# cc-ai/climategan

Hardware: AMD Instinct MI355X
Metric: 640x640 images/sec (G+D step): per-domain sample slots per second of the joint Masker+Painter training step (update_G + update_D), global batch 32 per domain (higher is better)
Workload: dtype bf16

## Files before the change

### climategan_amd/csrc/conv_wgrad.hip

```cpp
#include "cgan_common.h"
#include <type_traits>

namespace {


struct WgradArgs {
  const uint16_t* x;
  const uint16_t* dy;
  float* dw;
  unsigned x_bytes, dy_bytes;
  float* ws;
  float* bpart;
  int n, h_in, w_in, cin, cin_s;
  int cout, cout_s;
  int kh, kw, stride, pad, dil;
  int h_out, w_out, npix;
  int nchunks, ci_blocks, co_blocks, splits, per_xcd;
  int coop, co_pairs, n_pairs;
  int fold, cpt, tpt, tap_slots;
  CGAN_DEV_ONLY(int dbg;)
  int reflect;
  int x_ups;
  CGAN_DEV_ONLY(unsigned long long* ts;)
};
// ... 324 lines not shown
  const unsigned row_b = (unsigned)wx * cin_b;
  const wg_rsrc_t rs_x = wg_make_rsrc(p.x, p.x_bytes);
  const wg_rsrc_t rs_dy = wg_make_rsrc(p.dy, p.dy_bytes);
  unsigned dy_c = 0x80000000u;
  {
    const int co = (cop * G + mem) * 64 + q8;
    if ((cop * G + mem) < p.co_blocks && co < p.cout_s) dy_c = (unsigned)prow * cout_b + (unsigned)co * 2u;
  }
  int lx, ly;
  unsigned cch2, x_c;
  {
    int slot, cib, ky, kx, cch;
    bool ok = n_tile(mem, slot, cib);
    if (p.fold) {
      const int tl = qs / p.cpt, tap_l = slot * p.tpt + tl;
      ok = ok && tl < p.tpt && tap_l < taps_n;
      const int tcl = ok ? tap_l : 0;
      ky = tcl / p.kw;
      kx = tcl - ky * p.kw;
      cch = (qs - tl * p.cpt) * 8;
    } else {
      ky = slot / p.kw;
      kx = slot - ky * p.kw;
      cch = cib * 64 + q8;
      ok = ok && cch < p.cin_s;
    }
    const int tap_y = ky * p.dil - p.pad, tap_x = kx * p.dil - p.pad;
    const int lxr = prow * p.stride + tap_x;
    ly = tap_y;
    lx = ok ? lxr : -(1 << 20);
    cch2 = (unsigned)cch * 2u;
    x_c = (unsigned)((tap_y * wx + lxr) * (int)cin_b) + cch2;
  }

  int v_sx, v_sy, v_nh;
  {
    const int pix = split * CHUNK2 + (lane & (PPS - 1)) * 8;
    const int r = pix / p.w_out;
    v_sx = (pix - r * p.w_out) * p.stride;
    const int nn = r / p.h_out;
    v_sy = (r - nn * p.h_out) * p.stride;
    v_nh = nn * hx;
  }
  unsigned u_dy = (unsigned)(split * CHUNK2) * cout_b;
  const int step = p.splits * CHUNK2;
  const int step_r = step / p.w_out;
  const int step_sx = (step - step_r * p.w_out) * p.stride;
  const int step_n = step_r / p.h_out;
  const int step_sy = (step_r - step_n * p.h_out) * p.stride;
  const int step_nh = step_n * hx;
  const int wrap_x = p.w_out * p.stride, wrap_y = p.h_out * p.stride;
  const unsigned step_dy = (unsigned)step * cout_b;

  unsigned v_off = 0;
  auto issue_piece = [&](int b, int k) {
    unsigned char* dst = smem + b * STAGE2 + mem * SUB2 + half * (PW * PIECE);
    if (k < PW) {
      const unsigned off = u_dy + (unsigned)((half * PW + k) * 8) * cout_b + dy_c;
      wg_dma16(rs_dy, dst + k * PIECE, off);
      return;
    }
    const int j = k - PW, i = half * PW + j;
    if (j == 0) v_off = (unsigned)((v_nh + v_sy) * wx + v_sx) * cin_b;
    int iy = __builtin_amdgcn_readlane(v_sy, i) + ly, ix = __builtin_amdgcn_readlane(v_sx, i) + lx;
    if (MODE == 2) {
      iy = iy < 0 ? -iy : (iy >= p.h_in ? 2 * p.h_in - 2 - iy : iy);
      ix = ix < 0 ? -ix : (ix >= p.w_in ? 2 * p.w_in - 2 - ix : ix);
    }
    const bool xv = ((unsigned)iy < (unsigned)p.h_in) & ((unsigned)ix < (unsigned)p.w_in);
    unsigned off;
    if (MODE == 1) off = (unsigned)(__builtin_amdgcn_readlane(v_nh, i) + (iy >> 1)) * row_b + (unsigned)(ix >> 1) * cin_b + cch2;
    else if (MODE == 2) off = (unsigned)(__builtin_amdgcn_readlane(v_nh, i) + iy) * row_b + (unsigned)ix * cin_b + cch2;
    else off = (unsigned)__builtin_amdgcn_readlane((int)v_off, i) + x_c;
    wg_dma16(rs_x, dst + G * SUB2 + j * PIECE, xv ? off : 0xffffffffu);
  };
  auto advance = [&]() {
    u_dy += step_dy;
    int sx = v_sx + step_sx, sy = v_sy + step_sy, nh = v_nh + step_nh;
    const bool cx = sx >= wrap_x;
    sx = cx ? sx - wrap_x : sx;
    sy = cx ? sy + p.stride : sy;
    const bool cy = sy >= wrap_y;
    sy = cy ? sy - wrap_y : sy;
    nh = cy ? nh + hx : nh;
    v_sx = sx; v_sy = sy; v_nh = nh;
  };

  const int wc = wave % G, wn = wave / G;
  f32x4 acc[4][4];
#pragma unroll
  for (int a = 0; a < 4; ++a)
#pragma unroll
    for (int b = 0; b < 4; ++b) acc[a][b] = (f32x4){0.f, 0.f, 0.f, 0.f};

  const bool do_bias = BIAS && p.bpart != nullptr && np == 0 && wn == 0;
  f32x4 accb[4];
#pragma unroll
  for (int a = 0; a < 4; ++a) accb[a] = (f32x4){0.f, 0.f, 0.f, 0.f};
  const int nchunks = (p.npix + CHUNK2 - 1) / CHUNK2;
  int c = split, buf = 0;
  unsigned long long t_a = 0, t_b = 0, ts_sum[4] = {0, 0, 0, 0}, t_start = 0;
  if (TS) t_start = __builtin_readcyclecounter();
  if (c < nchunks) {
#pragma unroll
    for (int k = 0; k < 2 * PW; ++k) issue_piece(0, k);
    advance();
  }
  for (; c < nchunks; c += p.splits) {
    if (TS) t_a = __builtin_readcyclecounter();
    asm volatile("s_waitcnt vmcnt(0) lgkmcnt(0)" ::: "memory");
    if (TS) { t_b = __builtin_readcyclecounter(); ts_sum[0] += t_b - t_a; }
    __syncthreads();
    if (TS) { t_a = __builtin_readcyclecounter(); ts_sum[1] += t_a - t_b; }
    if (c + p.splits < nchunks) {
#pragma unroll
      for (int k = 0; k < 2 * PW; ++k) issue_piece(buf ^ 1, k);
      advance();
    }
    if (TS) { t_b = __builtin_readcyclecounter(); ts_sum[2] += t_b - t_a; }
    const unsigned char* sdy = smem + buf * STAGE2 + wc * SUB2;
    const unsigned char* sx = smem + buf * STAGE2 + (G + wn) * SUB2;
#pragma unroll
    for (int ks = 0; ks < CH / 32; ++ks) {
      u32x4 fa[4], fb[4];
#pragma unroll
      for (int a = 0; a < 4; ++a) fa[a] = tr_frag(sdy + ks * 4 * PIECE, a, lane);
#pragma unroll
      for (int b = 0; b < 4; ++b) fb[b] = tr_frag(sx + ks * 4 * PIECE, b, lane);
#pragma unroll
      for (int a = 0; a < 4; ++a)
#pragma unroll
        for (int b = 0; b < 4; ++b) acc[a][b] = mfma16(as_vec8<T>(fa[a]), as_vec8<T>(fb[b]), acc[a][b]);
      if (BIAS && do_bias) {
#pragma unroll
        for (int a = 0; a < 4; ++a) accb[a] = mfma16(as_vec8<T>(fa[a]), as_vec8<T>(ones_frag<T>()), accb[a]);
      }
    }
    buf ^= 1;
    if (TS) { t_a = __builtin_readcyclecounter(); ts_sum[3] += t_a - t_b; }
  }
  if (BIAS && do_bias && cop * G + wc < p.co_blocks)
    store_bias_row(p.bpart + (size_t)split * p.cout_s, accb, 4, (cop * G + wc) * 64, p.cout_s, lane);
  if (TS && CGAN_WTS(p) && lane == 0) {
    unsigned long long* o = CGAN_WTS(p) + ((size_t)blockIdx.x * (G * G) + wave) * 8;
    o[0] = t_start;
    o[1] = __builtin_readcyclecounter();
    for (int i = 0; i < 4; ++i) o[2 + i] = ts_sum[i];
    o[6] = (unsigned long long)((nchunks - split + p.splits - 1) / p.splits);
  }

  const int cob = cop * G + wc;
  int slot_c, cib_c;
  const bool nt_ok = n_tile(wn, slot_c, cib_c);
  if (cob >= p.co_blocks || !nt_ok) return;
  if (p.ws) {
    const int tiles_n = p.tap_slots * p.ci_blocks * p.co_blocks;
    const int tile = (slot_c * p.ci_blocks + cib_c) * p.co_blocks + cob;
    f32x4* wst = reinterpret_cast<f32x4*>(p.ws) + ((size_t)split * tiles_n + tile) * 1024;
#pragma unroll
    for (int a = 0; a < 4; ++a)
#pragma unroll
      for (int b = 0; b < 4; ++b) wst[(a * 4 + b) * 64 + lane] = acc[a][b];
    return;
  }
  const int j = lane & 15, g = lane >> 4;
#pragma unroll
  for (int b = 0; b < 4; ++b) {
    int tap, ci;
    const bool col_ok = wgrad_column(p.fold, p.cpt, p.tpt, taps_n, p.cin, slot_c, cib_c, b * 16 + j, tap, ci);
#pragma unroll
    for (int a = 0; a < 4; ++a)
#pragma unroll
      for (int r = 0; r < 4; ++r) {
        const int co = cob * 64 + a * 16 + 4 * g + r;
        if (co < p.cout && col_ok && !(CGAN_DBG(p) & 1)) atomicAdd(p.dw + ((size_t)co * p.cin + ci) * taps_n + tap, acc[a][b][r]);
      }
  }
}

constexpr int TL_W = 32, TL_H = 4, TL_XP = 40;
constexpr int TL_XH_BYTES = (TL_H + 2) * TL_XP * 128;
constexpr int TL_DY_BYTES = TL_H * TL_W * 128;

__device__ __forceinline__ u32x4 tr_frag_at(const unsigned char* slab, int q0, int tile, int lane) {
  const int i = lane & 15, g = lane >> 4;
  const int k = i >> 2;
  const int chunk = tile * 2 + ((i & 3) >> 1);
  const int qa = q0 + 8 * g + k, qb = qa + 4;
  const unsigned char* a0 = slab + qa * 128 + ((chunk ^ swz(qa & 7)) << 4) + (i & 1) * 8;
  const unsigned char* a1 = slab + qb * 128 + ((chunk ^ swz(qb & 7)) << 4) + (i & 1) * 8;
  s16x4 lo = __builtin_amdgcn_ds_read_tr16_b64_v4i16((__attribute__((address_space(3))) s16x4*)a0);
  s16x4 hi = __builtin_amdgcn_ds_read_tr16_b64_v4i16((__attribute__((address_space(3))) s16x4*)a1);
  u32x4 r;
  r[0] = (uint16_t)lo[0] | ((uint32_t)(uint16_t)lo[1] << 16);
  r[1] = (uint16_t)lo[2] | ((uint32_t)(uint16_t)lo[3] << 16);
  r[2] = (uint16_t)hi[0] | ((uint32_t)(uint16_t)hi[1] << 16);
  r[3] = (uint16_t)hi[2] | ((uint32_t)(uint16_t)hi[3] << 16);
  return r;
}

template <typename T, int NA = 4, bool BIAS = false>
__global__ __launch_bounds__(256, 2) void conv_wgrad_tile3x3_kernel(WgradArgs p) {
  extern __shared__ __attribute__((aligned(1024))) unsigned char smem[];
  unsigned char* xh = smem;
  unsigned char* dyt = smem + TL_XH_BYTES;
  const int lane = threadIdx.x & 63;
  const int wave = __builtin_amdgcn_readfirstlane(threadIdx.x >> 6);
  int item = (blockIdx.x & 7) * p.per_xcd + (blockIdx.x >> 3);
  if ((int)(blockIdx.x >> 3) >= p.per_xcd || item >= p.co_blocks * p.ci_blocks * p.splits) return;
  const int cob = item % p.co_blocks;
  item /= p.co_blocks;
  const int cib = item % p.ci_blocks;
  const int split = item / p.ci_blocks;

  const int prow = lane >> 3, qs = (lane & 7) ^ swz(prow);
  const unsigned cin_b = (unsigned)p.cin_s * 2u, cout_b = (unsigned)p.cout_s * 2u;
  const __amdgpu_buffer_rsrc_t rs_x = __builtin_amdgcn_make_buffer_rsrc(const_cast<uint16_t*>(p.x), 0, p.x_bytes, 0x00020000);
  const __amdgpu_buffer_rsrc_t rs_dy = __builtin_amdgcn_make_buffer_rsrc(const_cast<uint16_t*>(p.dy), 0, p.dy_bytes, 0x00020000);
  const bool ci_ok = cib * 64 + qs * 8 < p.cin_s, co_ok = cob * 64 + qs * 8 < p.cout_s;
  const unsigned x_c = (unsigned)(cib * 64 + qs * 8) * 2u, dy_c = (unsigned)(cob * 64 + qs * 8) * 2u;

  const int tw = p.w_out / TL_W, th = p.h_out / TL_H;
  const int ntiles = p.n * th * tw;

  auto stage = [&](int t) {
    const int tc = t % tw;
    const int r0 = t / tw;
    const int tr = r0 % th, img = r0 / th;
    const int ty0 = tr * TL_H, tx0 = tc * TL_W;
#pragma unroll
    for (int rr = 0; rr < 2; ++rr) {
      const int r = wave + 4 * rr;
      if (r < TL_H + 2) {
        const int iy = ty0 - 1 + r;
        const unsigned row_off = (unsigned)((img * p.h_in + iy) * p.w_in) * cin_b + x_c;
#pragma unroll
        for (int i5 = 0; i5 < 5; ++i5) {
          const int ix = tx0 - 4 + 8 * i5 + prow;
          const bool ok = ci_ok & ((unsigned)iy < (unsigned)p.h_in) & ((unsigned)ix < (unsigned)p.w_in);
          __builtin_amdgcn_raw_ptr_buffer_load_lds(rs_x, (__attribute__((address_space(3))) void*)(xh + (r * TL_XP + 8 * i5) * 128), 16,
                                                   ok ? row_off + (unsigned)ix * cin_b : 0xffffffffu, 0, 0, 0);
        }
      }
    }
    const int j0 = wave < 2 ? wave * 2 : 4 + (wave - 2) * 6, nj = wave < 2 ? 2 : 6;
#pragma unroll
    for (int jj = 0; jj < 6; ++jj) {
      if (jj < nj) {
        const int j = j0 + jj, r = j >> 2, c8 = (j & 3) * 8;
        const unsigned off = (unsigned)((img * p.h_out + ty0 + r) * p.w_out + tx0 + c8 + prow) * cout_b + dy_c;
        __builtin_amdgcn_raw_ptr_buffer_load_lds(rs_dy, (__attribute__((address_space(3))) void*)(dyt + (r * TL_W + c8) * 128), 16,
                                                 co_ok ? off : 0xffffffffu, 0, 0, 0);
      }
    }
  };

  f32x4 acc[NA][9];
#pragma unroll
  for (int a = 0; a < NA; ++a)
#pragma unroll
    for (int i = 0; i < 9; ++i) acc[a][i] = (f32x4){0.f, 0.f, 0.f, 0.f};

  const bool do_bias = BIAS && p.bpart != nullptr && cib == 0 && wave == 0;
  f32x4 accb[4];
#pragma unroll
  for (int a = 0; a < 4; ++a) accb[a] = (f32x4){0.f, 0.f, 0.f, 0.f};
  for (int t = split; t < ntiles; t += p.splits) {
    __syncthreads();
    stage(t);
    asm volatile("s_waitcnt vmcnt(0)" ::: "memory");
    __syncthreads();
#pragma unroll 1
    for (int ty = 0; ty < TL_H; ++ty) {
      u32x4 fa[NA];
#pragma unroll
      for (int a = 0; a < NA; ++a) fa[a] = tr_frag_at(dyt, ty * TL_W, a, lane);
      if (BIAS && do_bias) {
#pragma unroll
        for (int a = 0; a < NA; ++a) accb[a] = mfma16(as_vec8<T>(fa[a]), as_vec8<T>(ones_frag<T>()), accb[a]);
      }
#pragma unroll
      for (int i = 0; i < 9; ++i) {
        const int jn = wave * 9 + i, tap = jn >> 2, grp = jn & 3;
        const int ky = tap / 3, kx = tap - ky * 3;
        const u32x4 fb = tr_frag_at(xh, (ty + ky) * TL_XP + 3 + kx, grp, lane);
#pragma unroll
        for (int a = 0; a < NA; ++a) acc[a][i] = mfma16(as_vec8<T>(fa[a]), as_vec8<T>(fb), acc[a][i]);
      }
    }
  }

  if (BIAS && do_bias) store_bias_row(p.bpart + (size_t)split * p.cout_s, accb, NA, cob * 64, p.cout_s, lane);
  const int tiles_n = 9 * p.ci_blocks * p.co_blocks;
#pragma unroll
  for (int i = 0; i < 9; ++i) {
    const int jn = wave * 9 + i, tap = jn >> 2, grp = jn & 3;
    const int tile = (tap * p.ci_blocks + cib) * p.co_blocks + cob;
    f32x4* wst = reinterpret_cast<f32x4*>(p.ws) + ((size_t)split * tiles_n + tile) * 1024;
#pragma unroll
    for (int a = 0; a < 4; ++a) wst[(a * 4 + grp) * 64 + lane] = a < NA ? acc[a < NA ? a : 0][i] : (f32x4){0.f, 0.f, 0.f, 0.f};
  }
}

template <int KL>
__global__ __launch_bounds__(256) void wgrad_reduce_kernel(const f32x4* __restrict__ ws, float* __restrict__ dw,
                                                           int splits, int taps, int tap_slots, int ci_blocks,
                                                           int co_blocks, int cout, int cin, int fold, int cpt,
                                                           int tpt, int main_blocks, const float* __restrict__ bpart,
                                                           int bias_rows, int cout_s, float* __restrict__ dbias) {
  if ((int)blockIdx.x >= main_blocks) {
    __shared__ float bsum[16][17];
    const int c16 = (int)threadIdx.x & 15, rl = (int)threadIdx.x >> 4;
    const int ch = ((int)blockIdx.x - main_blocks) * 16 + c16;
    float a0 = 0.f, a1 = 0.f, a2 = 0.f, a3 = 0.f;
    if (ch < cout) {
      int r = rl;
      for (; r + 48 < bias_rows; r += 64) {
        a0 += bpart[(size_t)r * cout_s + ch];
        a1 += bpart[(size_t)(r + 16) * cout_s + ch];
        a2 += bpart[(size_t)(r + 32) * cout_s + ch];
        a3 += bpart[(size_t)(r + 48) * cout_s + ch];
      }
      for (; r < bias_rows; r += 16) a0 += bpart[(size_t)r * cout_s + ch];
    }
    bsum[rl][c16] = (a0 + a1) + (a2 + a3);
    __syncthreads();
    if (rl == 0 && ch < cout) {
      float acc = 0.f;
#pragma unroll
      for (int l = 0; l < 16; ++l) acc += bsum[l][c16];
      dbias[ch] += acc;
    }
    return;
  }
  constexpr int EL = 256 / KL;
  __shared__ f32x4 red[KL][EL];
  const int tiles_n = tap_slots * ci_blocks * co_blocks;
  const int el = threadIdx.x % EL, kl = threadIdx.x / EL;
  const int e = blockIdx.x * EL + el;
  f32x4 s = (f32x4){0.f, 0.f, 0.f, 0.f};
  if (e < tiles_n * 1024) {
    const size_t stride = (size_t)tiles_n * 1024;
#pragma unroll 4
    for (int sp = kl; sp < splits; sp += KL) {
      const f32x4 v = ws[(size_t)sp * stride + e];
      s[0] += v[0]; s[1] += v[1]; s[2] += v[2]; s[3] += v[3];
    }
  }
  if (KL > 1) {
    red[kl][el] = s;
    __syncthreads();
    if (kl != 0) return;
#pragma unroll
    for (int l = 1; l < KL; ++l) {
      const f32x4 v = red[l][el];
      s[0] += v[0]; s[1] += v[1]; s[2] += v[2]; s[3] += v[3];
    }
  }
  if (e >= tiles_n * 1024) return;
  int tile = e >> 10;
  const int frag = (e >> 6) & 15, lane = e & 63;
  const int cob = tile % co_blocks;
  tile /= co_blocks;
  const int cib = tile % ci_blocks, slot = tile / ci_blocks;
  int tap, ci;
  if (!wgrad_column(fold, cpt, tpt, taps, cin, slot, cib, (frag & 3) * 16 + (lane & 15), tap, ci)) return;
#pragma unroll
  for (int r = 0; r < 4; ++r) {
    const int co = cob * 64 + (frag >> 2) * 16 + 4 * (lane >> 4) + r;
    if (co >= cout) continue;
    dw[((size_t)co * cin + ci) * taps + tap] += s[r];
  }
}

template <typename T>
__global__ __launch_bounds__(256) void channel_sum_kernel(const uint16_t* __restrict__ x, float* __restrict__ out,
                                                          long npix, int cs, int c, float* __restrict__ part) {
  extern __shared__ __attribute__((aligned(16))) float sm_cs[];
  const int groups = cs / 8;
  const int ppb = blockDim.x / groups;
  const int gi = threadIdx.x % groups, pl = threadIdx.x / groups;
  float s[8] = {0.f, 0.f, 0.f, 0.f, 0.f, 0.f, 0.f, 0.f};
  if (pl < ppb) {
#pragma unroll 4
    for (long pix = (long)blockIdx.x * ppb + pl; pix < npix; pix += (long)gridDim.x * ppb) {
      const u32x4 v = *reinterpret_cast<const u32x4*>(x + pix * cs + gi * 8);
#pragma unroll
      for (int e = 0; e < 4; ++e) {
        float a, b;
        unpack2<T>(v[e], a, b);
        s[2 * e] += a;
        s[2 * e + 1] += b;
      }
    }
#pragma unroll
    for (int e = 0; e < 8; ++e) sm_cs[(pl * groups + gi) * 8 + e] = s[e];
  }
  __syncthreads();
  for (int ch = threadIdx.x; ch < groups * 8; ch += blockDim.x) {
    if (ch >= c) continue;
    float acc = 0.f;
    for (int l = 0; l < ppb; ++l) acc += sm_cs[l * groups * 8 + ch];
    if (part) part[(size_t)blockIdx.x * cs + ch] = acc;
    else atomicAdd(out + ch, acc);
  }
}

CGAN_KNOB(int, g_wgrad_target, 0);
CGAN_KNOB(int, g_wgrad_dbg, 0);
CGAN_KNOB(int, g_wgrad_coop_min_pix, 32768);
CGAN_KNOB(int, g_wgrad_coop_chunk, 0);
CGAN_KNOB(int, g_wgrad_slots, 512);
CGAN_KNOB(int, g_wgrad_tile, 1);
CGAN_KNOB(int, g_wgrad_coop_g, 0);
CGAN_KNOB(int, g_wgrad_bias_fused, 1);
CGAN_KNOB(int, g_wgrad_ws_cost_pct, 100);
CGAN_KNOB(unsigned long long*, g_wgrad_ts, nullptr);
}

#ifdef CGAN_DEV
extern "C" void cgan_debug_set_wgrad_tsbuf(void* p) { g_wgrad_ts = (unsigned long long*)p; }
extern "C" void cgan_debug_set_wgrad_bias_fused(int v) { g_wgrad_bias_fused = v; }
extern "C" void cgan_debug_set_wgrad_ws_cost(int pct) { g_wgrad_ws_cost_pct = pct > 0 ? pct : 100; }
extern "C" void cgan_debug_set_wgrad_tile3x3(int v) { g_wgrad_tile = v; }
extern "C" void cgan_debug_set_wgrad_slots(int v) { g_wgrad_slots = v > 0 ? v : 512; }
extern "C" void cgan_debug_set_wgrad_coop_chunk(int v) { g_wgrad_coop_chunk = (v == 32 || v == 64) ? v : 0; }

extern "C" void cgan_debug_set_wgrad_coop_min_pixels(int v) { g_wgrad_coop_min_pix = v; }
extern "C" void cgan_debug_set_wgrad_coop_g(int v) { g_wgrad_coop_g = (v == 2 || v == 4) ? v : 0; }

extern "C" void cgan_debug_set_wgrad(int target_workgroups, int dbg) {
  g_wgrad_target = target_workgroups;
  g_wgrad_dbg = dbg;
}
#endif

constexpr int BIAS_MAX_BLOCKS = 512;
constexpr int BIAS_MAX_ROWS = 1024;

struct WgradPlan {
  int fold, cpt, tpt, tap_slots, ci_blocks, co_blocks, splits;
  int coop, co_pairs, n_pairs, chunk;
  int g;
  int tile;
  long tiles() const { return (long)tap_slots * ci_blocks * co_blocks; }
};

static WgradPlan wgrad_plan(const CganConvDesc* d, bool have_ws = true) {
  WgradPlan pl;
  const int taps = d->kh * d->kw, cin_s = cgan_cs(d->c_in);
  pl.co_blocks = ceil_div(cgan_cs(d->c_out), 64);
  pl.fold = (cin_s <= 32 && taps > 1 && g_wgrad_dbg != 4) ? 1 : 0;
  pl.cpt = pl.fold ? cin_s / 8 : 8;
  pl.tpt = pl.fold ? 8 / pl.cpt : 1;
  pl.tap_slots = pl.fold ? ceil_div(taps, pl.tpt) : taps;
  pl.ci_blocks = pl.fold ? 1 : ceil_div(cin_s, 64);
  const long npix = (long)d->n * d->h_out * d->w_out;
  pl.g = 2;
  pl.co_pairs = (pl.co_blocks + 1) / 2;
  pl.n_pairs = pl.fold ? (pl.tap_slots + 1) / 2 : pl.tap_slots * ((pl.ci_blocks + 1) / 2);
  pl.coop = ((pl.co_blocks % 2) == 0 && ((pl.fold ? pl.tap_slots : pl.ci_blocks) % 2) == 0 && (d->w_out % 8) == 0 &&
             (g_wgrad_dbg & 8) == 0 && (double)npix * cgan_cs(d->c_out) * 2.0 < 1.9e9 &&
             (npix >= (long)g_wgrad_coop_min_pix || pl.tiles() >= 256))
                ? 1 : 0;
  pl.tile = ((g_wgrad_tile == 2 || (g_wgrad_tile == 1 && !pl.coop)) && have_ws && !pl.fold && d->kh == 3 && d->kw == 3 && d->stride == 1 && d->pad == 1 &&
             d->dilation == 1 && d->pad_mode == CGAN_PAD_ZERO && !d->in_upsample && (d->w_out % TL_W) == 0 &&
             (d->h_out % TL_H) == 0 && (cin_s % 64) == 0 && npix >= 65536 && (g_wgrad_dbg & (8 | 16)) == 0) ? 1 : 0;
  if (pl.tile) {
    pl.coop = 0;
    pl.chunk = TL_W * TL_H;
    const long pairs = (long)pl.co_blocks * pl.ci_blocks, ntiles = npix / (TL_W * TL_H);
    long sp = g_wgrad_target < 0 ? -g_wgrad_target : (long)g_wgrad_slots / pairs;
    if (sp > ntiles) sp = ntiles;
    pl.splits = sp < 1 ? 1 : (int)sp;
    return pl;
  }
  const long tiles = pl.coop ? (long)pl.co_pairs * pl.n_pairs : pl.tiles();
  auto plan_splits = [&](int chunk, long slots, int& nchunks_out) {
    const int nchunks = (int)((npix + chunk - 1) / chunk);
    nchunks_out = nchunks;
    long sp_best = 1;
    if (g_wgrad_target > 0) {
      sp_best = (g_wgrad_target + tiles - 1) / tiles;
    } else if (g_wgrad_target < 0) {
      sp_best = -g_wgrad_target;
    } else {
      const double t_ws = (pl.coop ? 0.024 : 0.008) * (g_wgrad_ws_cost_pct / 100.0);
      double best = 1e30;
      for (int m = 0; m <= 8; ++m) {
        long sp = m == 0 ? 1 : (slots * m) / tiles;
        if (sp < 1) continue;
        if (sp > nchunks) sp = nchunks;
        const long wgs = sp * tiles;
        const double cost = (double)((wgs + slots - 1) / slots) * ((double)((nchunks + sp - 1) / sp) + 2.0) + (double)wgs * t_ws;
        if (cost < best) { best = cost; sp_best = sp; }
      }
    }
    if (sp_best > nchunks) sp_best = nchunks;
    return sp_best < 1 ? 1L : sp_best;
  };
  int nchunks = 0;
  pl.chunk = pl.coop ? 64 : 128;
  if (pl.coop && g_wgrad_coop_g != 2 && (pl.co_blocks % 4) == 0 && ((pl.fold ? pl.tap_slots : pl.ci_blocks) % 4) == 0 &&
      g_wgrad_coop_chunk == 0) {
    const long tiles4 = (long)(pl.co_blocks / 4) * (pl.fold ? pl.tap_slots / 4 : (long)pl.tap_slots * (pl.ci_blocks / 4));
    const int nch = (int)((npix + 63) / 64);
    long sp = g_wgrad_target < 0 ? -g_wgrad_target : (g_wgrad_slots / 2) / tiles4;
    if (sp < 1) sp = 1;
    if (sp > nch) sp = nch;
    if (g_wgrad_coop_g == 4 || (tiles4 <= g_wgrad_slots / 2 && nch / sp >= 8)) {
      pl.g = 4;
      pl.co_pairs = pl.co_blocks / 4;
      pl.n_pairs = pl.fold ? pl.tap_slots / 4 : pl.tap_slots * (pl.ci_blocks / 4);
      pl.chunk = 64;
      pl.splits = (int)sp;
      return pl;
    }
  }
  long splits = plan_splits(pl.chunk, g_wgrad_slots, nchunks);
  if (pl.coop && (g_wgrad_coop_chunk == 32 || (g_wgrad_coop_chunk == 0 && nchunks / splits >= 96))) {
    pl.chunk = 32;
    splits = plan_splits(32, 2 * g_wgrad_slots, nchunks);
  }
  if (splits > nchunks) splits = nchunks;
  pl.splits = splits < 1 ? 1 : (int)splits;
  return pl;
}

extern "C" size_t cgan_conv2d_bwd_weight_workspace_bytes(const CganConvDesc* d) {
  if (!d || d->n <= 0 || d->h_out <= 0 || d->w_out <= 0 || d->c_in <= 0 || d->c_out <= 0 || d->kh <= 0 || d->kw <= 0)
    return 0;
  const WgradPlan pl = wgrad_plan(d);
  return (size_t)pl.tiles() * (size_t)pl.splits * 64 * 64 * sizeof(float) + (size_t)BIAS_MAX_ROWS * cgan_cs(d->c_out) * sizeof(float);
}

extern "C" int cgan_conv2d_nhwc_bwd_weight(const void* x, const void* dy, float* dw_oihw, float* dbias,
                                           const CganConvDesc* d, void* workspace, size_t workspace_bytes,
                                           void* stream) {
  CGAN_REQUIRE(d != nullptr && x && dy && dw_oihw, "conv2d_nhwc_bwd_weight: null pointer");
  CGAN_REQUIRE(d->dtype == CGAN_F16 || d->dtype == CGAN_BF16, "conv2d_nhwc_bwd_weight: bad dtype %d", d->dtype);
  CGAN_REQUIRE(d->pad_mode == CGAN_PAD_ZERO || d->pad_mode == CGAN_PAD_REFLECT, "conv2d_nhwc_bwd_weight: bad pad mode");
  if (d->pad_mode == CGAN_PAD_REFLECT)
    CGAN_REQUIRE(d->pad < d->h_in && d->pad < d->w_in && !d->in_upsample,
                 "conv2d_nhwc_bwd_weight: reflect padding must be < input size (and is not combined with in_upsample)");
  if (d->in_upsample) CGAN_REQUIRE((d->h_in % 2) == 0 && (d->w_in % 2) == 0, "conv2d_nhwc_bwd_weight: in_upsample needs even h_in/w_in");
  CGAN_REQUIRE(d->n > 0 && d->h_in > 0 && d->w_in > 0 && d->c_in > 0 && d->c_out > 0 && d->kh > 0 && d->kw > 0 &&
                   d->stride > 0 && d->dilation > 0 && d->pad >= 0,
               "conv2d_nhwc_bwd_weight: bad shape");
  const int eh = (d->h_in + 2 * d->pad - d->dilation * (d->kh - 1) - 1) / d->stride + 1;
  const int ew = (d->w_in + 2 * d->pad - d->dilation * (d->kw - 1) - 1) / d->stride + 1;
  CGAN_REQUIRE(eh == d->h_out && ew == d->w_out, "conv2d_nhwc_bwd_weight: h_out/w_out inconsistent");
  WgradArgs a;
  a.x = (const uint16_t*)x; a.dy = (const uint16_t*)dy; a.dw = dw_oihw;
  a.n = d->n; a.h_in = d->h_in; a.w_in = d->w_in; a.cin = d->c_in; a.cin_s = cgan_cs(d->c_in);
  a.cout = d->c_out; a.cout_s = cgan_cs(d->c_out);
  a.kh = d->kh; a.kw = d->kw; a.stride = d->stride; a.pad = d->pad; a.dil = d->dilation;
  a.h_out = d->h_out; a.w_out = d->w_out;
  const long npix = (long)d->n * d->h_out * d->w_out;
  CGAN_REQUIRE(npix < (1L << 31) - 256, "conv2d_nhwc_bwd_weight: too many pixels");
  a.npix = (int)npix;
  a.x_ups = d->in_upsample;
  a.reflect = d->pad_mode == CGAN_PAD_REFLECT;
  a.nchunks = ceil_div(a.npix, 128);
  const WgradPlan pl = wgrad_plan(d, workspace != nullptr);
  a.ci_blocks = pl.ci_blocks; a.co_blocks = pl.co_blocks; a.splits = pl.splits;
  a.fold = pl.fold; a.cpt = pl.cpt; a.tpt = pl.tpt; a.tap_slots = pl.tap_slots;
  a.coop = pl.coop; a.co_pairs = pl.co_pairs; a.n_pairs = pl.n_pairs;
  const int taps = d->kh * d->kw;
  CGAN_DEV_ONLY(a.dbg = g_wgrad_dbg; a.ts = g_wgrad_ts;)
  const long items = (long)a.splits * (pl.tile ? (long)pl.co_blocks * pl.ci_blocks
                                              : (pl.coop ? (long)pl.co_pairs * pl.n_pairs : pl.tiles()));
  a.per_xcd = (int)((items + 7) / 8);
  CGAN_REQUIRE(items < (1L << 30), "conv2d_nhwc_bwd_weight: grid too large");
  const unsigned gx = (unsigned)a.per_xcd * 8;
  a.ws = nullptr;
  a.bpart = nullptr;
  int bias_rows = 0;
  if (workspace) {
    CGAN_REQUIRE(workspace_bytes >= cgan_conv2d_bwd_weight_workspace_bytes(d),
                 "conv2d_nhwc_bwd_weight: workspace too small (%zu bytes)", workspace_bytes);
    a.ws = (float*)workspace;
    const int rows = a.splits * ((pl.tile || pl.coop) ? 1 : 4);
    const bool variant_ok = pl.tile ? (pl.co_blocks == 1 && ceil_div(cgan_cs(d->c_out), 16) < 4)
                                    : (!pl.coop || (pl.chunk == 64 && pl.g == 2));
    if (dbias && rows <= BIAS_MAX_ROWS && variant_ok && g_wgrad_bias_fused && CGAN_WTS(a) == nullptr) {
      a.bpart = a.ws + (size_t)pl.tiles() * (size_t)pl.splits * 64 * 64;
      bias_rows = rows;
    }
  }
  hipStream_t s = (hipStream_t)stream;
  const size_t smem = 4 * WAVE_LDS;
  CGAN_REQUIRE((double)d->n * (a.x_ups ? d->h_in / 2 : d->h_in) * (a.x_ups ? d->w_in / 2 : d->w_in) * a.cin_s * 2.0 < 4294967295.0 &&
                   (double)a.npix * a.cout_s * 2.0 < 4294967295.0,
               "conv2d_nhwc_bwd_weight: activation tensors of 4 GiB or more are not supported");
  a.x_bytes = (unsigned)((size_t)d->n * (a.x_ups ? d->h_in / 2 : d->h_in) * (a.x_ups ? d->w_in / 2 : d->w_in) * a.cin_s * 2);
  a.dy_bytes = (unsigned)((size_t)a.npix * a.cout_s * 2);
  const int mode = a.x_ups ? 1 : (a.reflect ? 2 : 0);
  const bool uni = (d->w_out % 8) == 0 && g_wgrad_dbg != 16 &&
                   ((double)a.npix + (double)a.splits * 128.0 + 128.0) * a.cout_s * 2.0 < 2147483648.0;
#define CGAN_BIG_LDS(KERNEL)                                                                                           \
  do {                                                                                                                 \
    static unsigned long long done_mask = 0;                                                                           \
    int dev_ = 0;                                                                                                      \
    (void)hipGetDevice(&dev_);                                                                                         \
    if (!((done_mask >> (dev_ & 63)) & 1ull)) {                                                                        \
      hipError_t e_ = hipFuncSetAttribute(reinterpret_cast<const void*>(&KERNEL),                                      \
                                          hipFuncAttributeMaxDynamicSharedMemorySize, 160 * 1024);                     \
      if (e_ != hipSuccess) {                                                                                          \
        cgan_set_error("conv2d_nhwc_bwd_weight: hipFuncSetAttribute failed: %s", hipGetErrorString(e_));               \
        return CGAN_ERR_HIP;                                                                                           \
      }                                                                                                                \
      done_mask |= 1ull << (dev_ & 63);                                                                                \
    }                                                                                                                  \
  } while (0)
#define WGRAD_LAUNCH(TT, MM, UU) do { CGAN_BIG_LDS((conv_wgrad_kernel<TT, MM, UU>)); hipLaunchKernelGGL((conv_wgrad_kernel<TT, MM, UU>), dim3(gx), dim3(256), smem, s, a); } while (0)
#define WGRAD_MODE(TT)                                                          \
  do {                                                                          \
    if (mode == 2) { if (uni) WGRAD_LAUNCH(TT, 2, true); else WGRAD_LAUNCH(TT, 2, false); }     \
    else if (mode == 1) { if (uni) WGRAD_LAUNCH(TT, 1, true); else WGRAD_LAUNCH(TT, 1, false); } \
    else { if (uni) WGRAD_LAUNCH(TT, 0, true); else WGRAD_LAUNCH(TT, 0, false); }                \
  } while (0)
  if (pl.tile) {
    const size_t smem3 = TL_XH_BYTES + TL_DY_BYTES;
    const int na = pl.co_blocks == 1 ? ceil_div(a.cout_s, 16) : 4;
#define TILE_LAUNCH(TT, NN, BB) hipLaunchKernelGGL((conv_wgrad_tile3x3_kernel<TT, NN, BB>), dim3(gx), dim3(256), smem3, s, a)
#define TILE_NB(TT, NN) do { if (a.bpart) TILE_LAUNCH(TT, NN, true); else TILE_LAUNCH(TT, NN, false); } while (0)
#define TILE_NA(TT) do { if (na == 1) TILE_NB(TT, 1); else if (na == 2) TILE_NB(TT, 2); else if (na == 3) TILE_NB(TT, 3); else TILE_LAUNCH(TT, 4, false); } while (0)
    if (d->dtype == CGAN_F16) TILE_NA(F16); else TILE_NA(BF16);
#undef TILE_NA
#undef TILE_NB
#undef TILE_LAUNCH
  } else if (pl.coop && pl.g == 4) {
    const size_t smem4 = (size_t)2 * 8 * 8 * PIECE;
#define COOP4_LAUNCH(TT, MM)                                                                                           \
  do {                                                                                                                 \
    CGAN_BIG_LDS((conv_wgrad_coop_kernel<TT, MM, 64, false, false, 4>));                                               \
    hipLaunchKernelGGL((conv_wgrad_coop_kernel<TT, MM, 64, false, false, 4>), dim3(gx), dim3(1024), smem4, s, a);      \
  } while (0)
#define COOP4_MODE(TT) do { if (mode == 1) COOP4_LAUNCH(TT, 1); else if (mode == 2) COOP4_LAUNCH(TT, 2); else COOP4_LAUNCH(TT, 0); } while (0)
#ifdef CGAN_DEV
    if (CGAN_WTS(a) && d->dtype == CGAN_BF16 && mode == 0) {
      CGAN_BIG_LDS((conv_wgrad_coop_kernel<BF16, 0, 64, true, false, 4>));
      hipLaunchKernelGGL((conv_wgrad_coop_kernel<BF16, 0, 64, true, false, 4>), dim3(gx), dim3(1024), smem4, s, a);
    } else
#endif
    if (d->dtype == CGAN_F16) COOP4_MODE(F16);
    else COOP4_MODE(BF16);
#undef COOP4_MODE
#undef COOP4_LAUNCH
  } else if (pl.coop) {
    const size_t smem2 = (size_t)2 * 4 * (pl.chunk / 8) * PIECE;
#define COOP_LAUNCH(TT, MM, CC, BB) do { CGAN_BIG_LDS((conv_wgrad_coop_kernel<TT, MM, CC, false, BB>)); hipLaunchKernelGGL((conv_wgrad_coop_kernel<TT, MM, CC, false, BB>), dim3(gx), dim3(256), smem2, s, a); } while (0)
#define COOP_MODE(TT)                                                                       \
  do {                                                                                      \
    if (pl.chunk == 32) { if (mode == 1) COOP_LAUNCH(TT, 1, 32, false); else if (mode == 2) COOP_LAUNCH(TT, 2, 32, false); else COOP_LAUNCH(TT, 0, 32, false); } \
    else if (a.bpart) { if (mode == 1) COOP_LAUNCH(TT, 1, 64, true); else if (mode == 2) COOP_LAUNCH(TT, 2, 64, true); else COOP_LAUNCH(TT, 0, 64, true); }            \
    else { if (mode == 1) COOP_LAUNCH(TT, 1, 64, false); else if (mode == 2) COOP_LAUNCH(TT, 2, 64, false); else COOP_LAUNCH(TT, 0, 64, false); }            \
  } while (0)
#ifdef CGAN_DEV
    if (CGAN_WTS(a) && d->dtype == CGAN_BF16 && mode == 0) {
      if (pl.chunk == 32) hipLaunchKernelGGL((conv_wgrad_coop_kernel<BF16, 0, 32, true>), dim3(gx), dim3(256), smem2, s, a);
      else { CGAN_BIG_LDS((conv_wgrad_coop_kernel<BF16, 0, 64, true>)); hipLaunchKernelGGL((conv_wgrad_coop_kernel<BF16, 0, 64, true>), dim3(gx), dim3(256), smem2, s, a); }
    } else
#endif
    if (d->dtype == CGAN_F16) COOP_MODE(F16);
    else COOP_MODE(BF16);
#undef COOP_MODE
#undef COOP_LAUNCH
  } else if (d->dtype == CGAN_F16) WGRAD_MODE(F16); else WGRAD_MODE(BF16);
#undef WGRAD_MODE
#undef WGRAD_LAUNCH
  CGAN_CHECK_LAUNCH("conv2d_nhwc_bwd_weight");
  float* bpart = a.bpart;
  if (dbias && !a.bpart) {
    const int cs = a.cout_s;
    const int threads = 256;
    const int ppb = threads / (cs / 8) > 0 ? threads / (cs / 8) : 1;
    CGAN_REQUIRE(cs / 8 <= threads, "conv2d_nhwc_bwd_weight: too many channels for the bias reduction");
    long want = (npix + (long)ppb * 16 - 1) / ((long)ppb * 16);
    const int grid = (int)(want < 1 ? 1 : (want > BIAS_MAX_BLOCKS ? BIAS_MAX_BLOCKS : want));
    const size_t smem_b = (size_t)ppb * (cs / 8) * 8 * sizeof(float);
    if (a.ws) {
      bpart = a.ws + (size_t)pl.tiles() * (size_t)pl.splits * 64 * 64;
      bias_rows = grid;
    }
    if (d->dtype == CGAN_F16)
      hipLaunchKernelGGL(channel_sum_kernel<F16>, dim3(grid), dim3(threads), smem_b, s, (const uint16_t*)dy, dbias, npix,
                         cs, d->c_out, bpart);
    else
      hipLaunchKernelGGL(channel_sum_kernel<BF16>, dim3(grid), dim3(threads), smem_b, s, (const uint16_t*)dy, dbias, npix,
                         cs, d->c_out, bpart);
    CGAN_CHECK_LAUNCH("conv2d_nhwc_bwd_weight(bias)");
  }
  if (a.ws) {
    const int elems = (int)pl.tiles() * 1024;
    const int bias_blocks = bpart ? ceil_div(d->c_out, 16) : 0;
    if (a.splits <= 4) {
      const int mb = ceil_div(elems, 256);
      hipLaunchKernelGGL(wgrad_reduce_kernel<1>, dim3(mb + bias_blocks), dim3(256), 0, s, (const f32x4*)a.ws, a.dw,
                         a.splits, taps, a.tap_slots, a.ci_blocks, a.co_blocks, a.cout, a.cin, a.fold, a.cpt, a.tpt, mb,
                         (const float*)bpart, bias_rows, a.cout_s, dbias);
    } else {
      const int mb = ceil_div(elems, 32);
      hipLaunchKernelGGL(wgrad_reduce_kernel<8>, dim3(mb + bias_blocks), dim3(256), 0, s, (const f32x4*)a.ws, a.dw,
                         a.splits, taps, a.tap_slots, a.ci_blocks, a.co_blocks, a.cout, a.cin, a.fold, a.cpt, a.tpt, mb,
                         (const float*)bpart, bias_rows, a.cout_s, dbias);
    }
    CGAN_CHECK_LAUNCH("conv2d_nhwc_bwd_weight(reduce)");
  }
  return CGAN_OK;
}
```

Measured before the change: 54.91.

## Add column-walking 3x3 wgrad kernel with row-ring input reuse

Adds a new 3x3 weight-gradient kernel in which each workgroup covers all input channels (64 or 128) for a group of up to five 16-wide output-channel tiles. It walks spatial tiles down a column and keeps input rows in an LDS ring buffer, so only the new rows are staged while the next tile is prefetched. The planner routes eligible shapes (large pixel counts, cin 128 with cout at least 40 by default) to this path and gives it its own split count and fused bias handling. The aim is less redundant input reloading and more MFMA work per staged byte, at the cost of large LDS use with one block per CU and fewer, longer-running workgroups.

```diff
diff --git a/climategan_amd/csrc/conv_wgrad.hip b/climategan_amd/csrc/conv_wgrad.hip
--- a/climategan_amd/csrc/conv_wgrad.hip
+++ b/climategan_amd/csrc/conv_wgrad.hip
@@ -650,6 +650,179 @@
   }
 }
 
+constexpr int CW_RING = 10, CW_NA_MAX = 5;
+constexpr int CW_ROW_BYTES = TL_XP * 128;
+constexpr int CW_PLANE_BYTES = CW_RING * CW_ROW_BYTES;
+constexpr int CW_DYBUF_BYTES = CW_NA_MAX * TL_H * 1024;
+constexpr int cw_lds_bytes(int cig) { return (cig / 4) * CW_PLANE_BYTES + 2 * CW_DYBUF_BYTES; }
+
+template <typename T, int NA, int CIG>
+__global__ __launch_bounds__(64 * CIG, 1) void conv_wgrad_col3x3_kernel(WgradArgs p) {
+  constexpr int NW = CIG, PLANES = CIG / 4;
+  constexpr int DYK = (NA * TL_H + NW - 1) / NW;
+  constexpr int NB = (NA + NW - 1) / NW;
+  extern __shared__ __attribute__((aligned(1024))) unsigned char smem[];
+  unsigned char* dyb = smem + PLANES * CW_PLANE_BYTES;
+  const int lane = threadIdx.x & 63;
+  const int wave = __builtin_amdgcn_readfirstlane(threadIdx.x >> 6);
+  int item = (blockIdx.x & 7) * p.per_xcd + (blockIdx.x >> 3);
+  if ((int)(blockIdx.x >> 3) >= p.per_xcd || item >= p.co_pairs * p.splits) return;
+  const int cg = item % p.co_pairs;
+  const int split = item / p.co_pairs;
+  const int cot_n = (p.cout_s + 15) >> 4;
+  const int ct0 = cg * NA + NA > cot_n ? cot_n - NA : cg * NA;
+  const int dup = cg * NA - ct0;
+
+  const int tw = p.w_out / TL_W, th = p.h_out / TL_H;
+  const long ntiles = (long)p.n * th * tw;
+  const int t_begin = (int)(ntiles * split / p.splits), t_end = (int)(ntiles * (split + 1) / p.splits);
+
+  const unsigned cin_b = (unsigned)p.cin_s * 2u, cout_b = (unsigned)p.cout_s * 2u;
+  const wg_rsrc_t rs_x = wg_make_rsrc(p.x, p.x_bytes);
+  const wg_rsrc_t rs_dy = wg_make_rsrc(p.dy, p.dy_bytes);
+  const int prow = lane >> 3, qs = (lane & 7) ^ swz(prow);
+  const int s_plane = wave % PLANES, s_row = wave / PLANES;
+  const unsigned x_c = (unsigned)(s_plane * 64 + qs * 8) * 2u;
+  const int dpos = lane >> 1;
+  const int dpx = (dpos & 3) | (((dpos >> 4) & 1) << 2) | (((dpos >> 2) & 3) << 3);
+  const int dch = (lane & 1) * 8;
+
+  auto stage = [&](int t, int b, int base, bool restart) {
+    const int tr = t % th, r0 = t / th;
+    const int tc = r0 % tw, img = r0 / tw;
+    const int ty0 = tr * TL_H, tx0 = tc * TL_W;
+#pragma unroll
+    for (int rr = 0; rr < 2; ++rr) {
+      if (rr == 1 && !(restart && s_row < 2)) continue;
+      const int j = rr == 0 ? 2 + s_row : s_row;
+      int slot = base + j;
+      slot = slot >= CW_RING ? slot - CW_RING : slot;
+      const int iy = ty0 - 1 + j;
+      const unsigned row_off = (unsigned)((img * p.h_in + iy) * p.w_in) * cin_b + x_c;
+      unsigned char* dst = smem + s_plane * CW_PLANE_BYTES + slot * CW_ROW_BYTES;
+#pragma unroll
+      for (int i5 = 0; i5 < 5; ++i5) {
+        const int ix = tx0 - 4 + 8 * i5 + prow;
+        const bool ok = ((unsigned)iy < (unsigned)p.h_in) & ((unsigned)ix < (unsigned)p.w_in);
+        wg_dma16(rs_x, dst + i5 * 1024, ok ? row_off + (unsigned)ix * cin_b : 0xffffffffu);
+      }
+    }
+#pragma unroll
+    for (int k = 0; k < DYK; ++k) {
+      const int pid = wave + NW * k, a = pid >> 2, ty = pid & 3;
+      if (a < NA) {
+        const int co = (ct0 + a) * 16 + dch;
+        const unsigned off = (unsigned)((img * p.h_out + ty0 + ty) * p.w_out + tx0 + dpx) * cout_b + (unsigned)co * 2u;
+        wg_dma16(rs_dy, dyb + b * CW_DYBUF_BYTES + pid * 1024, co < p.cout_s ? off : 0xffffffffu);
+      }
+    }
+  };
+
+  const int fi = lane & 15, fg = lane >> 4, fk = fi >> 2;
+  const int dy_lo = (4 * fg + fk) * 32 + (fi & 3) * 8;
+  const int c_plane = (wave >> 2) % PLANES, c_grp = wave & 3;
+  const unsigned char* xpl = smem + c_plane * CW_PLANE_BYTES;
+
+  f32x4 acc[NA][9];
+#pragma unroll
+  for (int a = 0; a < NA; ++a)
+#pragma unroll
+    for (int i = 0; i < 9; ++i) acc[a][i] = (f32x4){0.f, 0.f, 0.f, 0.f};
+  const bool do_bias = p.bpart != nullptr;
+  const bool bias_w = do_bias && wave < NA;
+  f32x4 accb[NB];
+#pragma unroll
+  for (int i = 0; i < NB; ++i) accb[i] = (f32x4){0.f, 0.f, 0.f, 0.f};
+
+  bool staged = false;
+  int base = 0;
+  for (int t = t_begin; t < t_end; ++t) {
+    const int buf = (t - t_begin) & 1;
+    if (!staged) {
+      asm volatile("s_waitcnt lgkmcnt(0)" ::: "memory");
+      __syncthreads();
+      base = 0;
+      stage(t, buf, 0, true);
+    }
+    asm volatile("s_waitcnt vmcnt(0) lgkmcnt(0)" ::: "memory");
+    __syncthreads();
+    staged = false;
+    if (t + 1 < t_end && ((t + 1) % th) != 0) {
+      int nb = base + TL_H;
+      nb = nb >= CW_RING ? nb - CW_RING : nb;
+      stage(t + 1, buf ^ 1, nb, false);
+      staged = true;
+    }
+    int rowoff[TL_H + 2];
+#pragma unroll
+    for (int j = 0; j < TL_H + 2; ++j) {
+      int s = base + j;
+      s = s >= CW_RING ? s - CW_RING : s;
+      rowoff[j] = s * CW_ROW_BYTES;
+    }
+    const unsigned char* dcur = dyb + buf * CW_DYBUF_BYTES;
+#pragma unroll
+    for (int ty = 0; ty < TL_H; ++ty) {
+      u32x4 fa[NA];
+#pragma unroll
+      for (int a = 0; a < NA; ++a) {
+        const unsigned char* a0 = dcur + (a * TL_H + ty) * 1024 + dy_lo;
+        s16x4 lo = __builtin_amdgcn_ds_read_tr16_b64_v4i16((__attribute__((address_space(3))) s16x4*)a0);
+        s16x4 hi = __builtin_amdgcn_ds_read_tr16_b64_v4i16((__attribute__((address_space(3))) s16x4*)(a0 + 512));
+        fa[a][0] = (uint16_t)lo[0] | ((uint32_t)(uint16_t)lo[1] << 16);
+        fa[a][1] = (uint16_t)lo[2] | ((uint32_t)(uint16_t)lo[3] << 16);
+        fa[a][2] = (uint16_t)hi[0] | ((uint32_t)(uint16_t)hi[1] << 16);
+        fa[a][3] = (uint16_t)hi[2] | ((uint32_t)(uint16_t)hi[3] << 16);
+      }
+      if (bias_w) {
+#pragma unroll
+        for (int i = 0; i < NB; ++i) {
+          u32x4 sel = fa[0];
+#pragma unroll
+          for (int aa = 1; aa < NA; ++aa) sel = (aa == wave + NW * i) ? fa[aa] : sel;
+          accb[i] = mfma16(as_vec8<T>(sel), as_vec8<T>(ones_frag<T>()), accb[i]);
+        }
+      }
+#pragma unroll
+      for (int tap = 0; tap < 9; ++tap) {
+        const int ky = tap / 3, kx = tap - ky * 3;
+        const u32x4 fb = tr_frag_at(xpl + rowoff[ty + ky], 3 + kx, c_grp, lane);
+#pragma unroll
+        for (int a = 0; a < NA; ++a) acc[a][tap] = mfma16(as_vec8<T>(fa[a]), as_vec8<T>(fb), acc[a][tap]);
+      }
+    }
+    if (staged) {
+      base += TL_H;
+      base = base >= CW_RING ? base - CW_RING : base;
+    }
+  }
+
+  if (do_bias && (lane & 15) == 0) {
+#pragma unroll
+    for (int i = 0; i < NB; ++i) {
+      const int a = wave + NW * i, co = (ct0 + a) * 16 + 4 * fg;
+      if (a < NA && a >= dup && co < p.cout_s) *reinterpret_cast<f32x4*>(p.bpart + (size_t)split * p.cout_s + co) = accb[i];
+    }
+  }
+  const int tiles_n = 9 * p.ci_blocks * p.co_blocks;
+  f32x4* wsp = reinterpret_cast<f32x4*>(p.ws) + (size_t)split * tiles_n * 1024;
+  const int pad_to = (cg == p.co_pairs - 1) ? p.co_blocks * 4 : 0;
+#pragma unroll
+  for (int tap = 0; tap < 9; ++tap) {
+#pragma unroll
+    for (int a = 0; a < NA; ++a) {
+      if (a < dup) continue;
+      const int ct = ct0 + a;
+      const int tile = (tap * p.ci_blocks + c_plane) * p.co_blocks + (ct >> 2);
+      wsp[(size_t)tile * 1024 + ((ct & 3) * 4 + c_grp) * 64 + lane] = acc[a][tap];
+    }
+    for (int ct = cot_n; ct < pad_to; ++ct) {
+      const int tile = (tap * p.ci_blocks + c_plane) * p.co_blocks + (ct >> 2);
+      wsp[(size_t)tile * 1024 + ((ct & 3) * 4 + c_grp) * 64 + lane] = (f32x4){0.f, 0.f, 0.f, 0.f};
+    }
+  }
+}
+
 template <int KL>
 __global__ __launch_bounds__(256) void wgrad_reduce_kernel(const f32x4* __restrict__ ws, float* __restrict__ dw,
                                                            int splits, int taps, int tap_slots, int ci_blocks,
@@ -791,6 +964,7 @@
   int coop, co_pairs, n_pairs, chunk;
   int g;
   int tile;
+  int col, co_groups, na;
   long tiles() const { return (long)tap_slots * ci_blocks * co_blocks; }
 };
 
@@ -811,6 +985,26 @@
              (g_wgrad_dbg & 8) == 0 && (double)npix * cgan_cs(d->c_out) * 2.0 < 1.9e9 &&
              (npix >= (long)g_wgrad_coop_min_pix || pl.tiles() >= 256))
                 ? 1 : 0;
+  const bool tiled_shape = have_ws && !pl.fold && d->kh == 3 && d->kw == 3 && d->stride == 1 && d->pad == 1 && d->dilation == 1 &&
+                           d->pad_mode == CGAN_PAD_ZERO && !d->in_upsample && (d->w_out % TL_W) == 0 && (d->h_out % TL_H) == 0 &&
+                           (g_wgrad_dbg & (8 | 16)) == 0;
+  pl.col = (tiled_shape && (cin_s == 64 || cin_s == 128) &&
+            (g_wgrad_tile == 3 || (npix >= 65536 && (g_wgrad_tile == 2 || (g_wgrad_tile == 1 && cin_s == 128 && cgan_cs(d->c_out) >= 40)))))
+               ? 1 : 0;
+  pl.co_groups = pl.na = 0;
+  pl.tile = 0;
+  if (pl.col) {
+    pl.coop = 0;
+    pl.chunk = TL_W * TL_H;
+    const int cot = ceil_div(cgan_cs(d->c_out), 16);
+    pl.co_groups = ceil_div(cot, CW_NA_MAX);
+    pl.na = ceil_div(cot, pl.co_groups);
+    const long ntiles = npix / (TL_W * TL_H);
+    long sp = g_wgrad_target < 0 ? -g_wgrad_target : (long)(g_wgrad_slots / 2) / pl.co_groups;
+    if (sp > ntiles) sp = ntiles;
+    pl.splits = sp < 1 ? 1 : (int)sp;
+    return pl;
+  }
   pl.tile = ((g_wgrad_tile == 2 || (g_wgrad_tile == 1 && !pl.coop)) && have_ws && !pl.fold && d->kh == 3 && d->kw == 3 && d->stride == 1 && d->pad == 1 &&
              d->dilation == 1 && d->pad_mode == CGAN_PAD_ZERO && !d->in_upsample && (d->w_out % TL_W) == 0 &&
              (d->h_out % TL_H) == 0 && (cin_s % 64) == 0 && npix >= 65536 && (g_wgrad_dbg & (8 | 16)) == 0) ? 1 : 0;
@@ -874,6 +1068,14 @@
   pl.splits = splits < 1 ? 1 : (int)splits;
   return pl;
 }
+
+#ifdef CGAN_DEV
+extern "C" int cgan_debug_wgrad_plan_kind(const CganConvDesc* d) {
+  if (!d) return -1;
+  const WgradPlan pl = wgrad_plan(d);
+  return pl.col ? 3 : (pl.tile ? 2 : (pl.coop ? 1 : 0));
+}
+#endif
 
 extern "C" size_t cgan_conv2d_bwd_weight_workspace_bytes(const CganConvDesc* d) {
   if (!d || d->n <= 0 || d->h_out <= 0 || d->w_out <= 0 || d->c_in <= 0 || d->c_out <= 0 || d->kh <= 0 || d->kw <= 0)
@@ -916,8 +1118,10 @@
   a.coop = pl.coop; a.co_pairs = pl.co_pairs; a.n_pairs = pl.n_pairs;
   const int taps = d->kh * d->kw;
   CGAN_DEV_ONLY(a.dbg = g_wgrad_dbg; a.ts = g_wgrad_ts;)
-  const long items = (long)a.splits * (pl.tile ? (long)pl.co_blocks * pl.ci_blocks
-                                              : (pl.coop ? (long)pl.co_pairs * pl.n_pairs : pl.tiles()));
+  if (pl.col) a.co_pairs = pl.co_groups;
+  const long items = (long)a.splits * (pl.col ? (long)pl.co_groups
+                                              : pl.tile ? (long)pl.co_blocks * pl.ci_blocks
+                                                        : (pl.coop ? (long)pl.co_pairs * pl.n_pairs : pl.tiles()));
   a.per_xcd = (int)((items + 7) / 8);
   CGAN_REQUIRE(items < (1L << 30), "conv2d_nhwc_bwd_weight: grid too large");
   const unsigned gx = (unsigned)a.per_xcd * 8;
@@ -928,8 +1132,8 @@
     CGAN_REQUIRE(workspace_bytes >= cgan_conv2d_bwd_weight_workspace_bytes(d),
                  "conv2d_nhwc_bwd_weight: workspace too small (%zu bytes)", workspace_bytes);
     a.ws = (float*)workspace;
-    const int rows = a.splits * ((pl.tile || pl.coop) ? 1 : 4);
-    const bool variant_ok = pl.tile ? (pl.co_blocks == 1 && ceil_div(cgan_cs(d->c_out), 16) < 4)
+    const int rows = a.splits * ((pl.col || pl.tile || pl.coop) ? 1 : 4);
+    const bool variant_ok = pl.col ? true : pl.tile ? (pl.co_blocks == 1 && ceil_div(cgan_cs(d->c_out), 16) < 4)
                                     : (!pl.coop || (pl.chunk == 64 && pl.g == 2));
     if (dbias && rows <= BIAS_MAX_ROWS && variant_ok && g_wgrad_bias_fused && CGAN_WTS(a) == nullptr) {
       a.bpart = a.ws + (size_t)pl.tiles() * (size_t)pl.splits * 64 * 64;
@@ -968,7 +1172,23 @@
     else if (mode == 1) { if (uni) WGRAD_LAUNCH(TT, 1, true); else WGRAD_LAUNCH(TT, 1, false); } \
     else { if (uni) WGRAD_LAUNCH(TT, 0, true); else WGRAD_LAUNCH(TT, 0, false); }                \
   } while (0)
-  if (pl.tile) {
+  if (pl.col) {
+#define COL_LAUNCH(TT, NN, GG)                                                                                         \
+  do {                                                                                                                 \
+    CGAN_BIG_LDS((conv_wgrad_col3x3_kernel<TT, NN, GG>));                                                              \
+    hipLaunchKernelGGL((conv_wgrad_col3x3_kernel<TT, NN, GG>), dim3(gx), dim3(64 * GG), cw_lds_bytes(GG), s, a);       \
+  } while (0)
+#define COL_NA(TT, GG)                                                                                                 \
+  do {                                                                                                                 \
+    if (pl.na == 1) COL_LAUNCH(TT, 1, GG); else if (pl.na == 2) COL_LAUNCH(TT, 2, GG); else if (pl.na == 3) COL_LAUNCH(TT, 3, GG); \
+    else if (pl.na == 4) COL_LAUNCH(TT, 4, GG); else COL_LAUNCH(TT, 5, GG);                                            \
+  } while (0)
+#define COL_CIG(TT) do { if (a.cin_s == 128) COL_NA(TT, 8); else COL_NA(TT, 4); } while (0)
+    if (d->dtype == CGAN_F16) COL_CIG(F16); else COL_CIG(BF16);
+#undef COL_CIG
+#undef COL_NA
+#undef COL_LAUNCH
+  } else if (pl.tile) {
     const size_t smem3 = TL_XH_BYTES + TL_DY_BYTES;
     const int na = pl.co_blocks == 1 ? ceil_div(a.cout_s, 16) : 4;
 #define TILE_LAUNCH(TT, NN, BB) hipLaunchKernelGGL((conv_wgrad_tile3x3_kernel<TT, NN, BB>), dim3(gx), dim3(256), smem3, s, a)
```

New measurement: 55.99 (median of 6 runs). 1.02x the previous value.
